# unclearness/vacancy

Hardware: AMD Instinct MI355X
Metric: Mvoxel*views/s (Carve) (higher is better)
Workload: dtype f32

## Files before the change

### include/vacancy_hip.h

```cpp
#ifndef VACANCY_HIP_H_
#define VACANCY_HIP_H_

#include <stdint.h>

#ifdef __cplusplus
extern "C" {
#endif

typedef enum vcy_status {
  VCY_OK = 0,
  VCY_ERR_INVALID_ARG = -1,
  VCY_ERR_NOT_INITIALIZED = -2,
  VCY_ERR_TOO_MANY_VOXELS = -3,
  VCY_ERR_HIP = -4,
  VCY_ERR_NO_DEVICE = -5,
  VCY_ERR_UNSUPPORTED = -6,
  VCY_ERR_INTERNAL = -7
} vcy_status;

enum { VCY_UPDATE_MAX = 0, VCY_UPDATE_WEIGHTED_AVERAGE = 1 };
enum { VCY_INTERP_NN = 0, VCY_INTERP_BILINEAR = 1 };
enum { VCY_OUTSIDE_NONE = 0, VCY_OUTSIDE_MAX = 1 };

typedef struct vcy_update_option {
// ... 127 lines not shown
int vcy_set_param(vcy_ctx* ctx, const char* name, int value);
int vcy_get_param(vcy_ctx* ctx, const char* name, int* value);
int vcy_set_stream(vcy_ctx* ctx, void* hip_stream);
int vcy_get_stream(vcy_ctx* ctx, void** hip_stream_out);
int vcy_sync(vcy_ctx* ctx);
int vcy_timer_begin(vcy_ctx* ctx);
int vcy_timer_end(vcy_ctx* ctx, float* elapsed_ms);

int vcy_last_carve_ms(vcy_ctx* ctx, float* prepass_ms, float* kernel_ms);
int vcy_carve_log(vcy_ctx* ctx, int max_records, float* begin_ms, float* prepass_ms, float* kernel_ms,
                  int32_t* first_chunk, int* n_records, int clear);

int vcy_last_carve_pairs(vcy_ctx* ctx, int64_t* processed, int64_t* total, int64_t* per_layer, int max_layers,
                         int* n_layers);

int vcy_plan_z_slabs(vcy_ctx* ctx, int n_views, const vcy_view* views, const float* const* sdf_device, int n_slabs,
                     int sample_stride, float brick_cost, int32_t* z_bounds, double* layer_cost, int max_layers,
                     int* n_layers);

int vcy_partition_layers(const double* layer_cost, int n_layers, int n_slabs, int nz, int32_t* z_bounds);

int vcy_selftest(vcy_ctx* ctx);

int vcy_measure_bandwidth(int device_id, uint64_t bytes, int reps, double* read_gbs, double* copy_gbs);

typedef struct vcy_clock_probe vcy_clock_probe;
int vcy_clock_probe_start(int device_id, int max_samples, vcy_clock_probe** out);
int vcy_clock_probe_stop(vcy_clock_probe* probe, double* mean_hz, double* settled_hz, double* min_hz, double* max_hz,
                         int* n_samples, double* covered_ms);

// ... 8 lines not shown
```

### vacancy_amd/capi.py

```python
import ctypes as C
import os

_HERE = os.path.dirname(os.path.abspath(__file__))
LIB_PATH = os.environ.get("VCY_HIP_LIB") or os.path.join(_HERE, "csrc", "libvacancy_hip.so")

VCY_OK, VCY_ERR_INVALID_ARG, VCY_ERR_NOT_INITIALIZED, VCY_ERR_TOO_MANY_VOXELS = 0, -1, -2, -3
VCY_ERR_HIP, VCY_ERR_NO_DEVICE, VCY_ERR_UNSUPPORTED, VCY_ERR_INTERNAL = -4, -5, -6, -7
VCY_UPDATE_MAX, VCY_UPDATE_WEIGHTED_AVERAGE = 0, 1
VCY_INTERP_NN, VCY_INTERP_BILINEAR = 0, 1
VCY_OUTSIDE_NONE, VCY_OUTSIDE_MAX = 0, 1


class UpdateOption(C.Structure):
    _fields_ = [
        ("voxel_update", C.c_int32),
        ("sdf_interp", C.c_int32),
        ("update_outside", C.c_int32),
        ("voxel_max_update_num", C.c_int32),
        ("voxel_update_weight", C.c_float),
        ("use_truncation", C.c_int32),
        ("truncation_band", C.c_float),
    ]

    def __init__(self, voxel_update=VCY_UPDATE_MAX, sdf_interp=VCY_INTERP_BILINEAR,
# ... 128 lines not shown
        "vcy_device_free": (C.c_int, [vp, vp]),
        "vcy_device_alloc": (C.c_int, [vp, C.c_int64, P(vp)]),
        "vcy_memcpy_h2d": (C.c_int, [vp, vp, vp, C.c_int64]),
        "vcy_memcpy_d2h": (C.c_int, [vp, vp, vp, C.c_int64]),
        "vcy_reset": (C.c_int, [vp]),
        "vcy_set_param": (C.c_int, [vp, C.c_char_p, C.c_int]),
        "vcy_get_param": (C.c_int, [vp, C.c_char_p, P(C.c_int)]),
        "vcy_set_stream": (C.c_int, [vp, vp]),
        "vcy_get_stream": (C.c_int, [vp, P(vp)]),
        "vcy_sync": (C.c_int, [vp]),
        "vcy_timer_begin": (C.c_int, [vp]),
        "vcy_timer_end": (C.c_int, [vp, P(C.c_float)]),
        "vcy_selftest": (C.c_int, [vp]),
        "vcy_last_carve_ms": (C.c_int, [vp, P(C.c_float), P(C.c_float)]),
        "vcy_last_carve_pairs": (C.c_int, [vp, P(C.c_int64), P(C.c_int64), vp, C.c_int, P(C.c_int)]),
        "vcy_plan_z_slabs": (C.c_int, [vp, C.c_int, P(View), P(vp), C.c_int, C.c_int, C.c_float, vp, vp, C.c_int,
                                       P(C.c_int)]),
        "vcy_last_stream_ms": (C.c_int, [vp, P(C.c_float), P(C.c_float), P(C.c_float)]),
        "vcy_partition_layers": (C.c_int, [vp, C.c_int, C.c_int, C.c_int, vp]),
        "vcy_carve_log": (C.c_int, [vp, C.c_int, vp, vp, vp, vp, P(C.c_int), C.c_int]),
        "vcy_measure_bandwidth": (C.c_int, [C.c_int, C.c_uint64, C.c_int, P(C.c_double), P(C.c_double)]),
        "vcy_clock_probe_start": (C.c_int, [C.c_int, C.c_int, P(vp)]),
        "vcy_clock_probe_stop": (C.c_int, [vp, P(C.c_double), P(C.c_double), P(C.c_double), P(C.c_double), P(C.c_int),
                                           P(C.c_double)]),
        "vcy_last_error": (C.c_char_p, []),
        "vcy_version": (C.c_char_p, []),
    }
    for name, (res, args) in sig.items():
        fn = getattr(lib, name)
        fn.restype = res
# ... 5 lines not shown
```

### vacancy_amd/carver.py

```python
import ctypes as C

import numpy as np

from . import capi
from .capi import CarverOption, Mesh, UpdateOption, View, make_view


def _p(a):
    return a.ctypes.data_as(C.c_void_p)


def _mesh_array(ptr, count, width, dtype):
    if count == 0 or not ptr:
        return np.zeros((0, width), dtype)
    return np.ctypeslib.as_array(ptr, shape=(count * width,)).reshape(count, width).copy()


def last_error():
    return capi.load().vcy_last_error().decode()


class VoxelCarver:
    def __init__(self, option=None, device_id=0, z_range=None):
        self._lib = capi.load()
# ... 277 lines not shown
    def selftest(self):
        return self._lib.vcy_selftest(self._ctx) == 0

    def last_carve_ms(self):
        a, b = C.c_float(), C.c_float()
        assert self._lib.vcy_last_carve_ms(self._ctx, C.byref(a), C.byref(b)) == 0, last_error()
        return a.value, b.value

    def last_carve_pairs(self):
        a, b, n = C.c_int64(), C.c_int64(), C.c_int()
        per = np.zeros(4096, np.int64)
        rc = self._lib.vcy_last_carve_pairs(self._ctx, C.byref(a), C.byref(b), _p(per), len(per), C.byref(n))
        if rc != 0:
            raise RuntimeError(last_error())
        return int(a.value), int(b.value), per[: n.value].copy()

    def plan_z_slabs(self, views, sdf_devs, n_slabs, stride=0, brick_cost=0.0):
        n, arr, ptrs = views if sdf_devs is None else self.prepare_batch(views, sdf_devs)
        bounds = np.zeros(n_slabs + 1, np.int32)
        cost = np.zeros(8192, np.float64)
        nl = C.c_int()
        rc = self._lib.vcy_plan_z_slabs(self._ctx, n, arr, ptrs, int(n_slabs), int(stride), float(brick_cost),
                                        _p(bounds), _p(cost), len(cost), C.byref(nl))
        if rc != 0:
            raise RuntimeError(last_error())
        return [int(z) for z in bounds], cost[: nl.value].copy()

    def carve_log(self, clear=True, max_records=8192):
        b = np.empty(max_records, np.float32)
        p = np.empty(max_records, np.float32)
# ... 168 lines not shown
```

### vacancy_amd/csrc/carve_fused.hip

```cpp
#include <algorithm>
#include <cmath>
#include <cstdlib>
#include <cstring>
#include <map>
#include <mutex>
#include <utility>
#include <type_traits>
#include <vector>

#include "carve_common.h"

namespace vcy {

void launch_fused_counts8(bool big, int update, bool trunc, bool samef, bool checkmax, unsigned grid_x, hipStream_t s,
                          const GridParams& g, const void* views, const float* c2, int nv, const ModeParams& m, int nbx, int nby,
                          int cull, int state_flags, const void* records, int64_t nbricks, float* bmin, const int* wgl,
                          unsigned long long* pcnt, int row_units);
void launch_fused_counts16(bool big, int update, bool trunc, bool samef, bool checkmax, unsigned grid_x, hipStream_t s,
                           const GridParams& g, const void* views, const float* c2, int nv, const ModeParams& m, int nbx, int nby,
                           int cull, int state_flags, const void* records, int64_t nbricks, float* bmin, const int* wgl,
                           unsigned long long* pcnt, int row_units);

namespace {

// ... 374 lines not shown
  const FusedView& fv = views[blockIdx.y];
  const int w = fv.v.width, h = fv.v.height, wq = (fv.wrect[2] - fv.wrect[0]) >> 2;
  const int t = blockIdx.x * 256 + threadIdx.x;
  if (fv.wmax == nullptr || wq <= 0 || t >= wq * (fv.wrect[3] - fv.wrect[1])) return;
  const int yr = t / wq, y = fv.wrect[1] + yr, x0 = fv.wrect[0] + ((t - yr * wq) << 2);
  const float* in = fv.wmax + (NEG ? 2 * (size_t)fv.wmax_plane : (size_t)0);
  const bool vec = (w & 3) == 0 && ((uintptr_t)in & 15) == 0;
  float a[8], b[8], o[4];
  wmax_load8(in + (size_t)y * w, x0, w, vec, a);
  wmax_load8(y + 4 < h ? in + (size_t)(y + 4) * w : nullptr, x0, w, vec, b);
#pragma unroll
  for (int j = 0; j < 4; ++j) o[j] = fmaxf(fmaxf(a[j], a[j + 4]), fmaxf(b[j], b[j + 4]));
  wmax_store4(const_cast<float*>(in) + (size_t)fv.wmax_plane + (size_t)y * w, x0, w, vec, o);
}

template <bool SAMEF, int TQ, bool GEN>
__device__ __forceinline__ TileInfo footprint_of(const FusedView& fv, float xl, float xh, float yl, float yh, float zl_,
                                                 float zh, bool is_ortho, bool outside_max, bool want_bound,
                                                 bool want_lower, float* lower_out = nullptr) {
  const ViewParams& v = fv.v;
  const float xa = fmaxf(fabsf(xl), fabsf(xh)), ya = fmaxf(fabsf(yl), fabsf(yh)), za = fmaxf(fabsf(zl_), fabsf(zh));
  const bool ortho = GEN && is_ortho;
  float p0[3], ax[3], ay[3], az[3], mag[3];
#pragma unroll
  for (int i = 0; i < 3; ++i) {
    p0[i] = v.t[i] + (v.r[i][0] * xl + (v.r[i][1] * yl + v.r[i][2] * zl_));
    ax[i] = v.r[i][0] * (xh - xl);
    ay[i] = v.r[i][1] * (yh - yl);
    az[i] = v.r[i][2] * (zh - zl_);
    mag[i] = fabsf(v.t[i]) + (fabsf(v.r[i][0]) * xa + (fabsf(v.r[i][1]) * ya + fabsf(v.r[i][2]) * za));
  }
  float umin = INFINITY, umax = -INFINITY, wmin = INFINITY, wmax_ = -INFINITY, zmin = INFINITY, zmax = -INFINITY;
  int bad = 0;
  const float fx = v.fx, fy = SAMEF ? v.fx : v.fy;
  float pxy[4][3];
// ... 26 lines not shown
  bad |= !(mag[0] < 0x1p60f) || !(mag[1] < 0x1p60f) || !(mag[2] < 0x1p60f);
  bad |= !(umin > -1.0e6f) || !(umax < 1.0e6f) || !(wmin > -1.0e6f) || !(wmax_ < 1.0e6f);
  const float uabs = fmaxf(fabsf(umin), fabsf(umax)), wabs = fmaxf(fabsf(wmin), fabsf(wmax_));
  float err_u, err_w;
  if (ortho) {
    err_u = 0x1p-21f * mag[0];
    err_w = 0x1p-21f * mag[1];
  } else {
    bad |= !(zmin * 4.0f >= zmax);
    const float iz = 0x1p-21f * __builtin_amdgcn_rcpf(zmin) * 1.0001f;
    err_u = iz * (fx * mag[0] + (uabs + fabsf(v.cx)) * mag[2]) + 0x1p-21f * (uabs + fabsf(v.cx));
    err_w = iz * (fy * mag[1] + (wabs + fabsf(v.cy)) * mag[2]) + 0x1p-21f * (wabs + fabsf(v.cy));
  }
  const float margin = 0.125f;
  bad |= !(err_u <= 0.03125f) || !(err_w <= 0.03125f);
  TileInfo ti;
  ti.lo_x = ti.lo_y = INFINITY;
  ti.hi_x = ti.hi_y = -INFINITY;
  ti.pitchf = 0.0f;
  ti.base = 0;
  ti.tx0 = ti.ty0 = ti.tw = ti.nq = ti.th = 0;
  ti.inv_tw = 1.0f;
  ti.ub = INFINITY;
  ti.sure = 0;
  if (!bad) {
    const int tx0 = max((int)floorf(umin - margin), v.roi_min_xi);
    const int ty0 = max((int)floorf(wmin - margin), v.roi_min_yi);
    const int tx1 = min((int)floorf(umax + margin), v.roi_max_xi);
    const int ty1 = min((int)floorf(wmax_ + margin), v.roi_max_yi);
    const int tw = tx1 - tx0 + 1, th = ty1 - ty0 + 1;
    constexpr bool kRaw = TQ == kTileRaw;
    if (tw > 0 && th > 0 && (kRaw ? (tw <= 15 && th <= 15) : ((tw + 1) * (th + 1) <= kBigPixels))) {
      const bool unclipped = (int)floorf(umin - margin) >= v.roi_min_xi && (int)floorf(wmin - margin) >= v.roi_min_yi &&
                             (int)floorf(umax + margin) < v.roi_max_xi && (int)floorf(wmax_ + margin) < v.roi_max_yi;
      const bool depth_ok = 0x1p-20f * mag[2] <= 0.25f * zmin && zmin >= 0x1p-58f && zmax <= 0x1p58f;
      const int pitch = kRaw ? 16 : tw + 1;
      const bool small_base = ty0 * pitch + tx0 < (1 << 18);
      const bool depth_ok_ortho = zmin > 0x1p-20f * mag[2];
      ti.sure = (unclipped && (ortho ? depth_ok_ortho : depth_ok) && small_base) ? 1 : 0;
      ti.tx0 = tx0;
      ti.ty0 = ty0;
      ti.tw = tw;
      ti.th = th;
      ti.nq = tw * th;
      ti.inv_tw = 1.0f / (float)pitch;
      ti.pitchf = (float)pitch;
      ti.base = -(ty0 * pitch + tx0);
      ti.lo_x = (float)tx0;
      ti.lo_y = (float)ty0;
      ti.hi_x = (tx1 == v.roi_max_xi) ? v.roi_max_x
                                      : __uint_as_float(__float_as_uint((float)(tx1 + 1)) - 1u);
      ti.hi_y = (ty1 == v.roi_max_yi) ? v.roi_max_y
                                      : __uint_as_float(__float_as_uint((float)(ty1 + 1)) - 1u);
      if (want_bound) {
        const int pw = min(tx1 + 1, v.roi_max_xi) - tx0 + 1;
        const int ph = min(ty1 + 1, v.roi_max_yi) - ty0 + 1;
        float m = -INFINITY;
        int has_nan = 0;
        gfloat_ptr wm = (gfloat_ptr)fv.wmax;
        const int L = min(pw, ph) >= 8 ? 3 : 2;
        const int k = 1 << L;
        const int nxw = (pw + k - 1) >> L, nyw = (ph + k - 1) >> L;
        const bool small = nxw <= 3 && nyw <= 3;
        const int ux = __any(small && nxw >= 3) ? 3 : (__any(small && nxw >= 2) ? 2 : 1);
        const int uy = __any(small && nyw >= 3) ? 3 : (__any(small && nyw >= 2) ? 2 : 1);
        if (wm != nullptr) {
          gfloat_ptr lvl = wm + (L == 3 ? (size_t)fv.wmax_plane : (size_t)0);
          const unsigned origin = __umul24((unsigned)v.width, (unsigned)ty0) + (unsigned)tx0 + (L == 3 ? (unsigned)fv.wmax_plane : 0u);
          if (nxw <= 3 && nyw <= 3) {
            float t[9];
#pragma unroll
            for (int bq = 0; bq < 3; ++bq) {
              const unsigned ro = origin + __umul24((unsigned)v.width, (unsigned)min(bq << L, max(ph - k, 0)));
#pragma unroll
              for (int aq = 0; aq < 3; ++aq) {
                t[3 * bq + aq] = -INFINITY;
                if (aq < ux && bq < uy) t[3 * bq + aq] = load_u32_index(wm, ro + (unsigned)min(aq << L, max(pw - k, 0)));
              }
            }
#pragma unroll
            for (int q = 0; q < 9; ++q) m = fmaxf(m, t[q]);
          } else {
            for (int bq = 0; bq < nyw; ++bq) {
              gfloat_ptr row = lvl + (unsigned)v.width * (unsigned)(ty0 + min(bq << L, max(ph - k, 0)));
              for (int aq = 0; aq < nxw; ++aq) m = fmaxf(m, row[tx0 + min(aq << L, max(pw - k, 0))]);
            }
          }
        } else {
          gfloat_ptr img = (gfloat_ptr)v.sdf;
          for (int j = 0; j < ph; ++j) {
            gfloat_ptr row = img + ((unsigned)v.width * (unsigned)(ty0 + j) + (unsigned)tx0);
            for (int i = 0; i < pw; ++i) {
              const float t = row[i];
              has_nan |= !(fabsf(t) <= 3.402823466e+38f);
              m = fmaxf(m, t);
            }
          }
        }
        if (outside_max && !ti.sure) {
          has_nan |= !(fabsf(v.max_sdf) <= 3.402823466e+38f);
          m = fmaxf(m, v.max_sdf);
        }
        ti.ub = has_nan ? INFINITY : (__builtin_fmaf(fabsf(m), 0x1p-20f, m) + 1.0e-30f);
        if (want_lower && ti.sure && !(ti.ub < -1.0f) && wm != nullptr && fv.has_lower && nxw <= 3 && nyw <= 3) {
          const unsigned origin = __umul24((unsigned)v.width, (unsigned)ty0) + (unsigned)tx0 +
                                  (L == 3 ? 3u : 2u) * (unsigned)fv.wmax_plane;
          float t[9], mneg = -INFINITY;
#pragma unroll
          for (int bq = 0; bq < 3; ++bq) {
            const unsigned ro = origin + __umul24((unsigned)v.width, (unsigned)min(bq << L, max(ph - k, 0)));
#pragma unroll
            for (int aq = 0; aq < 3; ++aq) {
              t[3 * bq + aq] = -INFINITY;
              if (aq < ux && bq < uy) t[3 * bq + aq] = load_u32_index(wm, ro + (unsigned)min(aq << L, max(pw - k, 0)));
            }
          }
#pragma unroll
          for (int q = 0; q < 9; ++q) mneg = fmaxf(mneg, t[q]);
          const float neg_lb = __builtin_fmaf(fabsf(mneg), 0x1p-20f, mneg);
          if (neg_lb <= 1.0f) ti.sure |= 2;
          if (lower_out) *lower_out = -neg_lb;
        }
      }
    }
  }
  return ti;
}

__device__ __forceinline__ FusedView load_fused_view(const FusedView* __restrict__ views, int vi) {
  static_assert(sizeof(FusedView) % 4 == 0, "FusedView is fetched dword by dword");
  constexpr int kViewDwords = (int)(sizeof(FusedView) / 4);
  typedef const uint32_t __attribute__((address_space(1))) * gu32_ptr;
  gu32_ptr src = (gu32_ptr)views + (size_t)vi * kViewDwords;
  uint32_t raw[kViewDwords];
#pragma unroll
  for (int q = 0; q < kViewDwords; ++q) raw[q] = src[q];
#pragma unroll
  for (int q = 0; q < kViewDwords; ++q) asm volatile("" : "+v"(raw[q]));
// ... 92 lines not shown
};
BlockDecode make_block_decode(unsigned grid_x, int nbx, int nby) {
  BlockDecode d;
  d.total = (int)grid_x;
  d.layer = nbx * nby;
  d.q = d.layer >> 3;
  d.rem = d.layer & 7;
  d.dealt = 8 * d.q * (int)(grid_x / (unsigned)std::max(d.layer, 1));
  d.dq = make_fast_div_u32((uint32_t)std::max(d.q, 1));
  d.drem = make_fast_div_u32((uint32_t)std::max(d.rem, 1));
  d.dnbx = make_fast_div_u32((uint32_t)std::max(nbx, 1));
  d.dnby = make_fast_div_u32((uint32_t)std::max(nby, 1));
  return d;
}

template <bool SAMEF, bool GEN>
__global__ __launch_bounds__(256) void footprint_records_kernel(GridParams g, const FusedView* __restrict__ views,
                                                                int nbw, int nby, int64_t nbricks, ModeParams mode,
                                                                int want_bound, int want_lower,
                                                                FootprintRecord* __restrict__ records,
                                                                FastDivU32 div_nbw, FastDivU32 div_nby, int small32) {
  const int64_t brick = (int64_t)blockIdx.x * 256 + threadIdx.x;
  if (brick >= nbricks) return;
  const int vi = blockIdx.y;
  int bxw, by, bz;
  if (small32) {
    const uint32_t b32 = (uint32_t)brick;
    const uint32_t rowb = fast_div_u32(b32, div_nbw);
    bxw = (int)(b32 - rowb * (uint32_t)nbw);
    const uint32_t zz = fast_div_u32(rowb, div_nby);
    by = (int)(rowb - zz * (uint32_t)nby);
    bz = (int)zz;
  } else {
    bxw = (int)(brick % nbw);
    const int64_t rowb = brick / nbw;
    by = (int)(rowb % nby);
    bz = (int)(rowb / nby);
  }
  const int x_lo = min(bxw * WX, g.nx - 1), x_hi = min(bxw * WX + WX - 1, g.nx - 1);
  const int y_hi = min(by * BY + BY - 1, g.ny - 1), z_hi = min(bz * BZ + BZ - 1, g.nz_local - 1);
  const FusedView& fv = views[vi];
  gfloat_ptr ax = (gfloat_ptr)g.px, ay = (gfloat_ptr)g.py, az = (gfloat_ptr)g.pz;
  const TileInfo ti = footprint_of<SAMEF, kTileRaw, GEN>(
      fv, load_u32_index(ax, (unsigned)x_lo), load_u32_index(ax, (unsigned)x_hi), load_u32_index(ay, (unsigned)(by * BY)),
      load_u32_index(ay, (unsigned)y_hi), load_u32_index(az, (unsigned)(g.z0 + bz * BZ)),
      load_u32_index(az, (unsigned)(g.z0 + z_hi)), mode.ortho != 0, mode.outside == VCY_OUTSIDE_MAX, want_bound != 0,
      want_lower != 0);
  records[(int64_t)vi * nbricks + brick] = pack_footprint(ti, fv.v);
}

constexpr int kLiveThreads = 1024;
constexpr int kLiveEntryWords = 2 + 2 * kWgWaves;
__global__ __launch_bounds__(kLiveThreads) void live_workgroups_kernel(const FootprintRecord* __restrict__ recs, int64_t nbricks,
                                                                       int nviews, const float* __restrict__ bmin, int trunc,
                                                                       int nbx, int nby, int nbw, int nwg, int* __restrict__ list,
                                                                       int unit_bricks, int entry_words) {
  __shared__ int wave_count[kLiveThreads / 64];
  __shared__ int block_base;
  const int wg = blockIdx.x * kLiveThreads + threadIdx.x;
  bool live = false;
  unsigned live_bricks = 0u;
  FootprintRecord rec0[kWgWaves];
  for (int j = 0; j < kWgWaves; ++j) rec0[j].w0 = 0u, rec0[j].w1 = 0u;
// ... 1368 lines not shown
  }
  const int row_views = c->row_kernel < 0 ? kRowMaxViews : std::min(c->row_kernel, kRowMaxViews);
  const bool rows = !big && !checkmax && (c->nx & (WX - 1)) == 0 && n_views <= row_views && c->prologue_mode != 1;
  const int nseg = (nbw + kRowBricks - 1) / kRowBricks;
  const bool one_view = c->one_view && n_views == 1 && !rows && !big && !checkmax && c->prologue_mode != 1;
  const bool coop_ok = (kWgWaves == 4 || kWgWaves == 8) && (c->nx & (WX - 1)) == 0 && !big && !rows;
  const int coop_views = c->fresh ? 1 : (u.voxel_update == VCY_UPDATE_MAX ? 1 : kLiveListMaxViews);
  const bool coop = coop_ok && (c->coop_store > 0 || (c->coop_store < 0 && n_views <= coop_views));
  const bool nt = coop && c->nt_store != 0;
  const int state_flags_base = (c->fresh ? 1 : 0) | (c->cnt_implied ? 2 : 0) | (c->brick_min_valid && !c->fresh ? 4 : 0) |
                               (coop ? 8 : 0) | (nt ? 16 : 0);
  const int64_t layer_bricks = (int64_t)nbw * nby;
  int chunk_layers = nbz;
  const int64_t rec_cap = c->record_bytes_max > 0 ? c->record_bytes_max : kRecordBytesMax;
  const bool in_kernel_prologue = !big && c->prologue_mode == 1;
  if (!big && !in_kernel_prologue) {
    const int64_t per_layer = layer_bricks * n_views * (int64_t)sizeof(FootprintRecord);
    const int64_t cap = rec_cap;
    chunk_layers = (int)std::max<int64_t>(1, std::min<int64_t>(nbz, cap / std::max<int64_t>(per_layer, 1)));
    const size_t need = (size_t)(per_layer * chunk_layers);
    if (c->records_bytes < need) {
      VCY_HIP_CHECK(hipStreamSynchronize(c->stream));
      if (c->d_records) (void)hipFree(c->d_records);
      c->d_records = nullptr;
      c->records_bytes = 0;
      VCY_HIP_CHECK(hipMalloc(&c->d_records, need));
      c->records_bytes = need;
    }
  }
  if (c->count_pairs) {
// ... 16 lines not shown
    gc.sdf = g.sdf + (int64_t)l0 * BZ * c->slice;
    gc.cnt = (char*)g.cnt + (int64_t)l0 * BZ * c->slice * c->cnt_bytes;
    gc.z0 = g.z0 + l0 * BZ;
    gc.nz_local = std::min(layers * BZ, nzl - l0 * BZ);
    const int64_t nbricks = layer_bricks * layers;
    FootprintRecord* recs = in_kernel_prologue ? nullptr : (FootprintRecord*)c->d_records;
    float* bmin = c->d_brick_min ? c->d_brick_min + (int64_t)l0 * layer_bricks : nullptr;
    unsigned long long* pcnt = c->count_pairs && c->d_pair_count ? c->d_pair_count + l0 : nullptr;
    if (timed && l0 > 0) {
      stamp = carve_log_open(c, false);
      if (stamp >= 0) VCY_HIP_CHECK(hipEventRecord(c->carve_log[stamp].ev[0], c->stream));
    }
    if (!big && !in_kernel_prologue) {
      const dim3 pgrid((unsigned)((nbricks + 255) / 256), (unsigned)n_views);
      const FastDivU32 div_nbw = make_fast_div_u32((uint32_t)nbw), div_nby = make_fast_div_u32((uint32_t)nby);
#define VCY_PREPASS(SF, GN)                                                                                       \
  hipLaunchKernelGGL((footprint_records_kernel<SF, GN>), pgrid, dim3(256), 0, c->stream, gc, d_views, nbw, nby,   \
                     nbricks, m, need_bound ? 1 : 0, want_lower ? 1 : 0, recs, div_nbw, div_nby,                  \
                     nbricks < 0xffffffffLL ? 1 : 0)
      if (samef) { if (gen) VCY_PREPASS(true, true); else VCY_PREPASS(true, false); }
      else { if (gen) VCY_PREPASS(false, true); else VCY_PREPASS(false, false); }
#undef VCY_PREPASS
      VCY_HIP_CHECK(hipGetLastError());
    }
    const int unit_bricks = rows ? kRowBricks : kWgWaves;
    const int units_x = rows ? nseg : nbx;
    const dim3 grid((unsigned)((int64_t)units_x * nby * layers));
    auto groups_of = [&](unsigned units) {
      return rows ? dim3((units + kRowWaves - 1) / kRowWaves) : dim3(units);
    };
    dim3 launch_grid = rows ? dim3(8u * ((grid.x + 8u * kRowWaves - 1) / (8u * kRowWaves))) : grid;
    const int* wgl = nullptr;
    int list_entry_words = 0;
    const bool have_min = u.voxel_update == VCY_UPDATE_MAX && (state_flags_base & 4) != 0 && bmin != nullptr;
    const bool list_pays = c->h_live_hint == nullptr || c->h_live_hint[1] <= 0 ||
                           (double)c->h_live_hint[0] < 0.6 * (double)c->h_live_hint[1];
    ++c->live_list_age;
    if (!big && recs != nullptr && c->use_live_list && need_bound && !c->fresh && n_views <= kLiveListMaxViews && (m.trunc != 0 || have_min) &&
// ... 186 lines not shown
```

### vacancy_amd/csrc/vcy_api.hip

```cpp
#include <algorithm>
#include <cstdarg>
#include <cstring>
#include <chrono>
#include <limits>
#include <mutex>
#include <thread>
#include <vector>

#include "vcy_internal.h"
#include "build_id.h"

namespace vcy {

static thread_local std::string g_last_error;

void set_error(const char* fmt, ...) {
  char buf[1024];
  va_list ap;
  va_start(ap, fmt);
  vsnprintf(buf, sizeof(buf), fmt, ap);
  va_end(ap);
  g_last_error = buf;
}

// ... 543 lines not shown
    return VCY_OK;
  }
  if (std::strcmp(name, "recordbytes") == 0) {
    c->record_bytes_max = value > 0 ? value : 0;
    return VCY_OK;
  }
  if (std::strcmp(name, "livelist") == 0) {
    c->use_live_list = value != 0;
    return VCY_OK;
  }
  if (std::strcmp(name, "prologue") == 0) {
    if (value < 0 || value > 2) return VCY_ERR_INVALID_ARG;
    c->prologue_mode = value;
    return VCY_OK;
  }
  if (std::strcmp(name, "livesync") == 0) {
    c->live_sync = value != 0;
    return VCY_OK;
  }
  if (std::strcmp(name, "coopstore") == 0) {
    c->coop_store = value < 0 ? -1 : (value != 0 ? 1 : 0);
    return VCY_OK;
  }
  if (std::strcmp(name, "listrecords") == 0) {
    c->list_records = value != 0;
    return VCY_OK;
  }
  if (std::strcmp(name, "eagerstate") == 0) {
    c->eager_state = value < 0 ? -1 : (value != 0 ? 1 : 0);
    return VCY_OK;
// ... 42 lines not shown
  else if (std::strcmp(name, "cull") == 0) *value = c->use_cull ? 1 : 0;
  else if (std::strcmp(name, "tile") == 0) *value = c->tile_mode;
  else if (std::strcmp(name, "defer") == 0) *value = c->defer ? 1 : 0;
  else if (std::strcmp(name, "shortdiv") == 0) *value = c->use_short_div ? 1 : 0;
  else if (std::strcmp(name, "div_level") == 0) *value = c->last_div_level;
  else if (std::strcmp(name, "mcsweep") == 0) *value = c->mc_sweep ? 1 : 0;
  else if (std::strcmp(name, "mcskip") == 0) *value = c->mc_skip;
  else if (std::strcmp(name, "rowkernel") == 0) *value = c->row_kernel;
  else if (std::strcmp(name, "ntstore") == 0) *value = c->nt_store;
  else if (std::strcmp(name, "oneview") == 0) *value = c->one_view;
  else if (std::strcmp(name, "eagerstate") == 0) *value = c->eager_state;
  else if (std::strcmp(name, "listrecords") == 0) *value = c->list_records;
  else if (std::strcmp(name, "mcdirect") == 0) *value = (int)std::min<int64_t>(c->mc_direct_bytes, 0x7fffffff);
  else if (std::strcmp(name, "livelist") == 0) *value = c->use_live_list ? 1 : 0;
  else if (std::strcmp(name, "prologue") == 0) *value = c->prologue_mode;
  else if (std::strcmp(name, "coopstore") == 0) *value = c->coop_store;
  else if (std::strcmp(name, "livesync") == 0) *value = c->live_sync ? 1 : 0;
  else if (std::strcmp(name, "brick_min_valid") == 0) *value = c->brick_min_valid && !c->fresh ? 1 : 0;
  else if (std::strcmp(name, "meshkeys") == 0) *value = c->mesh_keys ? 1 : 0;
  else if (std::strcmp(name, "lazycount") == 0) *value = c->lazy_count ? 1 : 0;
  else if (std::strcmp(name, "carvetimer") == 0) *value = c->time_carve ? 1 : 0;
  else if (std::strcmp(name, "carvelog_dropped") == 0) *value = c->carve_log_dropped;
  else if (std::strcmp(name, "count_bytes") == 0) *value = c->cnt_bytes;
  else if (std::strcmp(name, "count_bytes_final") == 0) *value = c->cnt_bytes_wire;
  else {
    set_error("unknown parameter %s", name);
    return VCY_ERR_INVALID_ARG;
  }
  return VCY_OK;
}
// ... 79 lines not shown
    return VCY_ERR_INVALID_ARG;
  }
  VCY_HIP_CHECK(hipSetDevice(c->device));
  const int nbz = (c->nz_local() + 7) / 8;
  std::vector<unsigned long long> h((size_t)nbz, 0ull);
  VCY_HIP_CHECK(hipMemcpyAsync(h.data(), c->d_pair_count, sizeof(unsigned long long) * (size_t)nbz, hipMemcpyDeviceToHost, c->stream));
  VCY_HIP_CHECK(hipStreamSynchronize(c->stream));
  int64_t sum = 0;
  for (int l = 0; l < nbz; ++l) {
    sum += (int64_t)h[(size_t)l];
    if (per_layer && l < max_layers) per_layer[l] = (int64_t)h[(size_t)l];
  }
  if (processed) *processed = sum;
  if (total) *total = (int64_t)((c->nx + 7) / 8) * ((c->ny + 7) / 8) * nbz * c->pair_count_views;
  if (n_layers) *n_layers = nbz;
  return VCY_OK;
}

int vcy_partition_layers(const double* layer_cost, int n_layers, int n_slabs, int nz, int32_t* z_bounds) {
  if (!layer_cost || !z_bounds || n_layers < 1 || n_slabs < 1 || n_slabs > n_layers || nz <= (n_layers - 1) * 8 ||
      nz > n_layers * 8) {
    set_error("vcy_partition_layers: invalid argument");
    return VCY_ERR_INVALID_ARG;
  }
  if (n_slabs > 1 && n_layers > 1 && nz - (n_layers - 1) * 8 == 1 && n_slabs > n_layers - 1) {
    set_error("vcy_partition_layers: the last layer is a single slice and cannot be a slab of its own");
    return VCY_ERR_INVALID_ARG;
  }
  for (int l = 0; l < n_layers; ++l)
    if (!(layer_cost[l] >= 0.0) || !(layer_cost[l] < 1e280)) {
// ... 888 lines not shown
```

### vacancy_amd/csrc/vcy_internal.h

```cpp
#pragma once

#include <hip/hip_runtime.h>

#include <cstdint>
#include <cstdio>
#include <string>
#include <utility>
#include <vector>

#include "vacancy_hip.h"

namespace vcy {

void set_error(const char* fmt, ...);

#define VCY_HIP_CHECK(expr)                                                        \
  do {                                                                             \
    hipError_t _e = (expr);                                                        \
    if (_e != hipSuccess) {                                                        \
      ::vcy::set_error("%s failed: %s (%s:%d)", #expr, hipGetErrorString(_e),      \
                       __FILE__, __LINE__);                                        \
      return VCY_ERR_HIP;                                                          \
    }                                                                              \
  } while (0)
// ... 79 lines not shown
  std::vector<CarveStamp> carve_log;
  int carve_log_n = 0;
  int carve_log_last = 0;
  int carve_log_dropped = 0;
  bool carve_log_last_dropped = false;
  int* h_live_hint = nullptr;
  int64_t live_list_age = 0;
  bool use_live_list = true;
  bool live_sync = true;
  int coop_store = -1;
  bool count_pairs = false;
  unsigned long long* d_pair_count = nullptr;
  int pair_count_layers = 0, pair_count_views = 0;
  int64_t record_bytes_max = 0;
  int prologue_mode = 0;
  void* d_records = nullptr;
  size_t records_bytes = 0;
  float* d_wmax = nullptr;
  size_t wmax_bytes = 0;
  bool fused_ortho = false;
  void* h_fused_stage[2] = {nullptr, nullptr};
  hipEvent_t ev_fused_stage[2] = {nullptr, nullptr};
  size_t fused_stage_bytes = 0;
  int fused_stage_idx = 0;
  bool fused_cache_valid = false;
  std::vector<char> fused_cache_vp;
  const float* fused_cache_wmax = nullptr;
  void* fused_cache_at = nullptr;
  bool fused_cache_bound = false, fused_cache_lower = false, fused_cache_ortho = false, fused_cache_samef = true;
  int fused_cache_max_quads = 0;
  int fused_cache_z[2] = {0, 0};
  void* d_stream_pool = nullptr;
// ... 73 lines not shown
```

Baseline: 4.286 million.

## Process two views per thread in footprint prepass to batch window loads

Adds a prepass kernel variant where each thread handles a brick for two views at once. It decodes the brick and loads its extent once, then issues both views' max-window loads before reducing them, so more independent memory loads are in flight per thread. The footprint code is split into helpers to support this, and the new variant is the default, selectable through a 'prepass' parameter. It also adds a debug API for copying records back to the host. In exchange the kernel uses more registers per thread and the grid has half as many view blocks.

New measurement: 4.339 million, median of 6. 1.01x the previous value.

```diff
diff --git a/include/vacancy_hip.h b/include/vacancy_hip.h
--- a/include/vacancy_hip.h
+++ b/include/vacancy_hip.h
@@ -165,6 +165,8 @@
 int vcy_last_carve_pairs(vcy_ctx* ctx, int64_t* processed, int64_t* total, int64_t* per_layer, int max_layers,
                          int* n_layers);
 
+int vcy_debug_copy_records(vcy_ctx* ctx, void* dst, int64_t max_bytes, int64_t* bytes);
+
 int vcy_plan_z_slabs(vcy_ctx* ctx, int n_views, const vcy_view* views, const float* const* sdf_device, int n_slabs,
                      int sample_stride, float brick_cost, int32_t* z_bounds, double* layer_cost, int max_layers,
                      int* n_layers);
diff --git a/vacancy_amd/capi.py b/vacancy_amd/capi.py
--- a/vacancy_amd/capi.py
+++ b/vacancy_amd/capi.py
@@ -166,6 +166,7 @@
         "vcy_selftest": (C.c_int, [vp]),
         "vcy_last_carve_ms": (C.c_int, [vp, P(C.c_float), P(C.c_float)]),
         "vcy_last_carve_pairs": (C.c_int, [vp, P(C.c_int64), P(C.c_int64), vp, C.c_int, P(C.c_int)]),
+        "vcy_debug_copy_records": (C.c_int, [vp, vp, C.c_int64, P(C.c_int64)]),
         "vcy_plan_z_slabs": (C.c_int, [vp, C.c_int, P(View), P(vp), C.c_int, C.c_int, C.c_float, vp, vp, C.c_int,
                                        P(C.c_int)]),
         "vcy_last_stream_ms": (C.c_int, [vp, P(C.c_float), P(C.c_float), P(C.c_float)]),
diff --git a/vacancy_amd/carver.py b/vacancy_amd/carver.py
--- a/vacancy_amd/carver.py
+++ b/vacancy_amd/carver.py
@@ -315,6 +315,18 @@
         if rc != 0:
             raise RuntimeError(last_error())
         return int(a.value), int(b.value), per[: n.value].copy()
+
+    def debug_records(self):
+        n = C.c_int64()
+        rc = self._lib.vcy_debug_copy_records(self._ctx, None, 0, C.byref(n))
+        if rc != 0:
+            raise RuntimeError(last_error())
+        out = np.zeros((n.value // 8, 2), np.uint32)
+        got = C.c_int64()
+        rc = self._lib.vcy_debug_copy_records(self._ctx, _p(out), out.nbytes, C.byref(got))
+        if rc != 0 or got.value != n.value:
+            raise RuntimeError(last_error())
+        return out
 
     def plan_z_slabs(self, views, sdf_devs, n_slabs, stride=0, brick_cost=0.0):
         n, arr, ptrs = views if sdf_devs is None else self.prepare_batch(views, sdf_devs)
diff --git a/vacancy_amd/csrc/carve_fused.hip b/vacancy_amd/csrc/carve_fused.hip
--- a/vacancy_amd/csrc/carve_fused.hip
+++ b/vacancy_amd/csrc/carve_fused.hip
@@ -412,11 +412,10 @@
   wmax_store4(const_cast<float*>(in) + (size_t)fv.wmax_plane + (size_t)y * w, x0, w, vec, o);
 }
 
+
 template <bool SAMEF, int TQ, bool GEN>
-__device__ __forceinline__ TileInfo footprint_of(const FusedView& fv, float xl, float xh, float yl, float yh, float zl_,
-                                                 float zh, bool is_ortho, bool outside_max, bool want_bound,
-                                                 bool want_lower, float* lower_out = nullptr) {
-  const ViewParams& v = fv.v;
+__device__ __forceinline__ bool footprint_rect(const ViewParams& v, float xl, float xh, float yl, float yh, float zl_,
+                                               float zh, bool is_ortho, TileInfo& ti, int& tx1_out, int& ty1_out) {
   const float xa = fmaxf(fabsf(xl), fabsf(xh)), ya = fmaxf(fabsf(yl), fabsf(yh)), za = fmaxf(fabsf(zl_), fabsf(zh));
   const bool ortho = GEN && is_ortho;
   float p0[3], ax[3], ay[3], az[3], mag[3];
@@ -473,7 +472,6 @@
   }
   const float margin = 0.125f;
   bad |= !(err_u <= 0.03125f) || !(err_w <= 0.03125f);
-  TileInfo ti;
   ti.lo_x = ti.lo_y = INFINITY;
   ti.hi_x = ti.hi_y = -INFINITY;
   ti.pitchf = 0.0f;
@@ -482,6 +480,7 @@
   ti.inv_tw = 1.0f;
   ti.ub = INFINITY;
   ti.sure = 0;
+  tx1_out = ty1_out = 0;
   if (!bad) {
     const int tx0 = max((int)floorf(umin - margin), v.roi_min_xi);
     const int ty0 = max((int)floorf(wmin - margin), v.roi_min_yi);
@@ -511,76 +510,125 @@
                                       : __uint_as_float(__float_as_uint((float)(tx1 + 1)) - 1u);
       ti.hi_y = (ty1 == v.roi_max_yi) ? v.roi_max_y
                                       : __uint_as_float(__float_as_uint((float)(ty1 + 1)) - 1u);
-      if (want_bound) {
-        const int pw = min(tx1 + 1, v.roi_max_xi) - tx0 + 1;
-        const int ph = min(ty1 + 1, v.roi_max_yi) - ty0 + 1;
-        float m = -INFINITY;
-        int has_nan = 0;
-        gfloat_ptr wm = (gfloat_ptr)fv.wmax;
-        const int L = min(pw, ph) >= 8 ? 3 : 2;
-        const int k = 1 << L;
-        const int nxw = (pw + k - 1) >> L, nyw = (ph + k - 1) >> L;
-        const bool small = nxw <= 3 && nyw <= 3;
-        const int ux = __any(small && nxw >= 3) ? 3 : (__any(small && nxw >= 2) ? 2 : 1);
-        const int uy = __any(small && nyw >= 3) ? 3 : (__any(small && nyw >= 2) ? 2 : 1);
-        if (wm != nullptr) {
-          gfloat_ptr lvl = wm + (L == 3 ? (size_t)fv.wmax_plane : (size_t)0);
-          const unsigned origin = __umul24((unsigned)v.width, (unsigned)ty0) + (unsigned)tx0 + (L == 3 ? (unsigned)fv.wmax_plane : 0u);
-          if (nxw <= 3 && nyw <= 3) {
-            float t[9];
-#pragma unroll
-            for (int bq = 0; bq < 3; ++bq) {
-              const unsigned ro = origin + __umul24((unsigned)v.width, (unsigned)min(bq << L, max(ph - k, 0)));
-#pragma unroll
-              for (int aq = 0; aq < 3; ++aq) {
-                t[3 * bq + aq] = -INFINITY;
-                if (aq < ux && bq < uy) t[3 * bq + aq] = load_u32_index(wm, ro + (unsigned)min(aq << L, max(pw - k, 0)));
-              }
-            }
-#pragma unroll
-            for (int q = 0; q < 9; ++q) m = fmaxf(m, t[q]);
-          } else {
-            for (int bq = 0; bq < nyw; ++bq) {
-              gfloat_ptr row = lvl + (unsigned)v.width * (unsigned)(ty0 + min(bq << L, max(ph - k, 0)));
-              for (int aq = 0; aq < nxw; ++aq) m = fmaxf(m, row[tx0 + min(aq << L, max(pw - k, 0))]);
-            }
-          }
-        } else {
-          gfloat_ptr img = (gfloat_ptr)v.sdf;
-          for (int j = 0; j < ph; ++j) {
-            gfloat_ptr row = img + ((unsigned)v.width * (unsigned)(ty0 + j) + (unsigned)tx0);
-            for (int i = 0; i < pw; ++i) {
-              const float t = row[i];
-              has_nan |= !(fabsf(t) <= 3.402823466e+38f);
-              m = fmaxf(m, t);
-            }
-          }
-        }
-        if (outside_max && !ti.sure) {
-          has_nan |= !(fabsf(v.max_sdf) <= 3.402823466e+38f);
-          m = fmaxf(m, v.max_sdf);
-        }
-        ti.ub = has_nan ? INFINITY : (__builtin_fmaf(fabsf(m), 0x1p-20f, m) + 1.0e-30f);
-        if (want_lower && ti.sure && !(ti.ub < -1.0f) && wm != nullptr && fv.has_lower && nxw <= 3 && nyw <= 3) {
-          const unsigned origin = __umul24((unsigned)v.width, (unsigned)ty0) + (unsigned)tx0 +
-                                  (L == 3 ? 3u : 2u) * (unsigned)fv.wmax_plane;
-          float t[9], mneg = -INFINITY;
-#pragma unroll
-          for (int bq = 0; bq < 3; ++bq) {
-            const unsigned ro = origin + __umul24((unsigned)v.width, (unsigned)min(bq << L, max(ph - k, 0)));
-#pragma unroll
-            for (int aq = 0; aq < 3; ++aq) {
-              t[3 * bq + aq] = -INFINITY;
-              if (aq < ux && bq < uy) t[3 * bq + aq] = load_u32_index(wm, ro + (unsigned)min(aq << L, max(pw - k, 0)));
-            }
-          }
-#pragma unroll
-          for (int q = 0; q < 9; ++q) mneg = fmaxf(mneg, t[q]);
-          const float neg_lb = __builtin_fmaf(fabsf(mneg), 0x1p-20f, mneg);
-          if (neg_lb <= 1.0f) ti.sure |= 2;
-          if (lower_out) *lower_out = -neg_lb;
-        }
-      }
+      tx1_out = tx1;
+      ty1_out = ty1;
+      return true;
+    }
+  }
+  return false;
+}
+
+struct WindowPlan {
+  int L, pw, ph, nxw, nyw;
+};
+__device__ __forceinline__ WindowPlan window_plan(const ViewParams& v, int tx0, int ty0, int tx1, int ty1) {
+  WindowPlan p;
+  p.pw = min(tx1 + 1, v.roi_max_xi) - tx0 + 1;
+  p.ph = min(ty1 + 1, v.roi_max_yi) - ty0 + 1;
+  p.L = min(p.pw, p.ph) >= 8 ? 3 : 2;
+  const int k = 1 << p.L;
+  p.nxw = (p.pw + k - 1) >> p.L;
+  p.nyw = (p.ph + k - 1) >> p.L;
+  return p;
+}
+
+__device__ __forceinline__ void window_loads(gfloat_ptr wm, unsigned origin, unsigned width, const WindowPlan& p,
+                                             int ux, int uy, bool on, float t[9]) {
+  const int k = 1 << p.L;
+#pragma unroll
+  for (int bq = 0; bq < 3; ++bq) {
+    const unsigned ro = origin + __umul24(width, (unsigned)min(bq << p.L, max(p.ph - k, 0)));
+#pragma unroll
+    for (int aq = 0; aq < 3; ++aq) {
+      t[3 * bq + aq] = -INFINITY;
+      if (aq < ux && bq < uy) t[3 * bq + aq] = load_u32_index(wm, on ? ro + (unsigned)min(aq << p.L, max(p.pw - k, 0)) : 0u);
+    }
+  }
+}
+
+__device__ __forceinline__ void window_counts(const WindowPlan& p, bool small, int& ux, int& uy) {
+  ux = __any(small && p.nxw >= 3) ? 3 : (__any(small && p.nxw >= 2) ? 2 : 1);
+  uy = __any(small && p.nyw >= 3) ? 3 : (__any(small && p.nyw >= 2) ? 2 : 1);
+}
+
+__device__ __forceinline__ float window_max_slow(const FusedView& fv, int tx0, int ty0, const WindowPlan& p, int* has_nan) {
+  const ViewParams& v = fv.v;
+  gfloat_ptr wm = (gfloat_ptr)fv.wmax;
+  float m = -INFINITY;
+  if (wm != nullptr) {
+    const int k = 1 << p.L;
+    gfloat_ptr lvl = wm + (p.L == 3 ? (size_t)fv.wmax_plane : (size_t)0);
+    for (int bq = 0; bq < p.nyw; ++bq) {
+      gfloat_ptr row = lvl + (unsigned)v.width * (unsigned)(ty0 + min(bq << p.L, max(p.ph - k, 0)));
+      for (int aq = 0; aq < p.nxw; ++aq) m = fmaxf(m, row[tx0 + min(aq << p.L, max(p.pw - k, 0))]);
+    }
+  } else {
+    gfloat_ptr img = (gfloat_ptr)v.sdf;
+    for (int j = 0; j < p.ph; ++j) {
+      gfloat_ptr row = img + ((unsigned)v.width * (unsigned)(ty0 + j) + (unsigned)tx0);
+      for (int i = 0; i < p.pw; ++i) {
+        const float t = row[i];
+        *has_nan |= !(fabsf(t) <= 3.402823466e+38f);
+        m = fmaxf(m, t);
+      }
+    }
+  }
+  return m;
+}
+
+__device__ __forceinline__ float footprint_ub(const ViewParams& v, float m, int has_nan, bool outside_max, int sure) {
+  if (outside_max && !sure) {
+    has_nan |= !(fabsf(v.max_sdf) <= 3.402823466e+38f);
+    m = fmaxf(m, v.max_sdf);
+  }
+  return has_nan ? INFINITY : (__builtin_fmaf(fabsf(m), 0x1p-20f, m) + 1.0e-30f);
+}
+
+__device__ __forceinline__ bool wants_lower(const FusedView& fv, const TileInfo& ti, const WindowPlan& p) {
+  return ti.sure && !(ti.ub < -1.0f) && fv.wmax != nullptr && fv.has_lower && p.nxw <= 3 && p.nyw <= 3;
+}
+__device__ __forceinline__ unsigned lower_origin(const FusedView& fv, int tx0, int ty0, const WindowPlan& p) {
+  return __umul24((unsigned)fv.v.width, (unsigned)ty0) + (unsigned)tx0 + (p.L == 3 ? 3u : 2u) * (unsigned)fv.wmax_plane;
+}
+__device__ __forceinline__ float neg_lower_bound(const float t[9]) {
+  float mneg = -INFINITY;
+#pragma unroll
+  for (int q = 0; q < 9; ++q) mneg = fmaxf(mneg, t[q]);
+  return __builtin_fmaf(fabsf(mneg), 0x1p-20f, mneg);
+}
+
+template <bool SAMEF, int TQ, bool GEN>
+__device__ __forceinline__ TileInfo footprint_of(const FusedView& fv, float xl, float xh, float yl, float yh, float zl_,
+                                                 float zh, bool is_ortho, bool outside_max, bool want_bound,
+                                                 bool want_lower, float* lower_out = nullptr) {
+  const ViewParams& v = fv.v;
+  TileInfo ti;
+  int tx1, ty1;
+  if (footprint_rect<SAMEF, TQ, GEN>(v, xl, xh, yl, yh, zl_, zh, is_ortho, ti, tx1, ty1) && want_bound) {
+    const int tx0 = ti.tx0, ty0 = ti.ty0;
+    const WindowPlan p = window_plan(v, tx0, ty0, tx1, ty1);
+    float m = -INFINITY;
+    int has_nan = 0;
+    gfloat_ptr wm = (gfloat_ptr)fv.wmax;
+    const bool small = p.nxw <= 3 && p.nyw <= 3;
+    int ux, uy;
+    window_counts(p, small, ux, uy);
+    if (wm != nullptr && small) {
+      float t[9];
+      window_loads(wm, __umul24((unsigned)v.width, (unsigned)ty0) + (unsigned)tx0 + (p.L == 3 ? (unsigned)fv.wmax_plane : 0u),
+                   (unsigned)v.width, p, ux, uy, true, t);
+#pragma unroll
+      for (int q = 0; q < 9; ++q) m = fmaxf(m, t[q]);
+    } else {
+      m = window_max_slow(fv, tx0, ty0, p, &has_nan);
+    }
+    ti.ub = footprint_ub(v, m, has_nan, outside_max, ti.sure);
+    if (want_lower && wants_lower(fv, ti, p)) {
+      float t[9];
+      window_loads(wm, lower_origin(fv, tx0, ty0, p), (unsigned)v.width, p, ux, uy, true, t);
+      const float neg_lb = neg_lower_bound(t);
+      if (neg_lb <= 1.0f) ti.sure |= 2;
+      if (lower_out) *lower_out = -neg_lb;
     }
   }
   return ti;
@@ -703,16 +751,8 @@
   return d;
 }
 
-template <bool SAMEF, bool GEN>
-__global__ __launch_bounds__(256) void footprint_records_kernel(GridParams g, const FusedView* __restrict__ views,
-                                                                int nbw, int nby, int64_t nbricks, ModeParams mode,
-                                                                int want_bound, int want_lower,
-                                                                FootprintRecord* __restrict__ records,
-                                                                FastDivU32 div_nbw, FastDivU32 div_nby, int small32) {
-  const int64_t brick = (int64_t)blockIdx.x * 256 + threadIdx.x;
-  if (brick >= nbricks) return;
-  const int vi = blockIdx.y;
-  int bxw, by, bz;
+__device__ __forceinline__ void decode_brick(int64_t brick, int nbw, int nby, FastDivU32 div_nbw, FastDivU32 div_nby,
+                                             int small32, int& bxw, int& by, int& bz) {
   if (small32) {
     const uint32_t b32 = (uint32_t)brick;
     const uint32_t rowb = fast_div_u32(b32, div_nbw);
@@ -726,16 +766,118 @@
     by = (int)(rowb % nby);
     bz = (int)(rowb / nby);
   }
+}
+
+__device__ __forceinline__ void brick_extent(const GridParams& g, int bxw, int by, int bz, float ext[6]) {
   const int x_lo = min(bxw * WX, g.nx - 1), x_hi = min(bxw * WX + WX - 1, g.nx - 1);
   const int y_hi = min(by * BY + BY - 1, g.ny - 1), z_hi = min(bz * BZ + BZ - 1, g.nz_local - 1);
+  gfloat_ptr ax = (gfloat_ptr)g.px, ay = (gfloat_ptr)g.py, az = (gfloat_ptr)g.pz;
+  ext[0] = load_u32_index(ax, (unsigned)x_lo);
+  ext[1] = load_u32_index(ax, (unsigned)x_hi);
+  ext[2] = load_u32_index(ay, (unsigned)(by * BY));
+  ext[3] = load_u32_index(ay, (unsigned)y_hi);
+  ext[4] = load_u32_index(az, (unsigned)(g.z0 + bz * BZ));
+  ext[5] = load_u32_index(az, (unsigned)(g.z0 + z_hi));
+}
+
+template <bool SAMEF, bool GEN>
+__global__ __launch_bounds__(256) void footprint_records_kernel(GridParams g, const FusedView* __restrict__ views,
+                                                                int nbw, int nby, int64_t nbricks, ModeParams mode,
+                                                                int want_bound, int want_lower,
+                                                                FootprintRecord* __restrict__ records,
+                                                                FastDivU32 div_nbw, FastDivU32 div_nby, int small32) {
+  const int64_t brick = (int64_t)blockIdx.x * 256 + threadIdx.x;
+  if (brick >= nbricks) return;
+  const int vi = blockIdx.y;
+  int bxw, by, bz;
+  decode_brick(brick, nbw, nby, div_nbw, div_nby, small32, bxw, by, bz);
   const FusedView& fv = views[vi];
-  gfloat_ptr ax = (gfloat_ptr)g.px, ay = (gfloat_ptr)g.py, az = (gfloat_ptr)g.pz;
-  const TileInfo ti = footprint_of<SAMEF, kTileRaw, GEN>(
-      fv, load_u32_index(ax, (unsigned)x_lo), load_u32_index(ax, (unsigned)x_hi), load_u32_index(ay, (unsigned)(by * BY)),
-      load_u32_index(ay, (unsigned)y_hi), load_u32_index(az, (unsigned)(g.z0 + bz * BZ)),
-      load_u32_index(az, (unsigned)(g.z0 + z_hi)), mode.ortho != 0, mode.outside == VCY_OUTSIDE_MAX, want_bound != 0,
-      want_lower != 0);
+  float e[6];
+  brick_extent(g, bxw, by, bz, e);
+  const TileInfo ti = footprint_of<SAMEF, kTileRaw, GEN>(fv, e[0], e[1], e[2], e[3], e[4], e[5], mode.ortho != 0,
+                                                         mode.outside == VCY_OUTSIDE_MAX, want_bound != 0, want_lower != 0);
   records[(int64_t)vi * nbricks + brick] = pack_footprint(ti, fv.v);
+}
+
+constexpr int kPrepassViews = 2;
+
+template <bool SAMEF, bool GEN, int VT>
+__global__ __launch_bounds__(256) void footprint_records_vt_kernel(GridParams g, const FusedView* __restrict__ views,
+                                                                   int nviews, int nbw, int nby, int64_t nbricks,
+                                                                   ModeParams mode, int want_bound, int want_lower,
+                                                                   FootprintRecord* __restrict__ records,
+                                                                   FastDivU32 div_nbw, FastDivU32 div_nby, int small32) {
+  const int64_t brick = (int64_t)blockIdx.x * 256 + threadIdx.x;
+  if (brick >= nbricks) return;
+  const int v0 = blockIdx.y * VT;
+  const int nv = min(VT, nviews - v0);
+  int bxw, by, bz;
+  decode_brick(brick, nbw, nby, div_nbw, div_nby, small32, bxw, by, bz);
+  float e[6];
+  brick_extent(g, bxw, by, bz, e);
+  TileInfo ti[VT];
+  WindowPlan p[VT];
+  bool has[VT];
+#pragma unroll
+  for (int k = 0; k < VT; ++k) {
+    if (k < nv) {
+      const ViewParams& v = views[v0 + k].v;
+      int tx1, ty1;
+      has[k] = footprint_rect<SAMEF, kTileRaw, GEN>(v, e[0], e[1], e[2], e[3], e[4], e[5], mode.ortho != 0, ti[k], tx1, ty1);
+      p[k] = window_plan(v, ti[k].tx0, ti[k].ty0, tx1, ty1);
+    }
+  }
+  if (want_bound) {
+    float t[VT][9];
+    int ux[VT], uy[VT];
+#pragma unroll
+    for (int k = 0; k < VT; ++k) {
+      if (k < nv) {
+        const FusedView& fv = views[v0 + k];
+        const bool small = has[k] && p[k].nxw <= 3 && p[k].nyw <= 3;
+        window_counts(p[k], small, ux[k], uy[k]);
+        if (fv.wmax != nullptr)
+          window_loads((gfloat_ptr)fv.wmax,
+                       __umul24((unsigned)fv.v.width, (unsigned)ti[k].ty0) + (unsigned)ti[k].tx0 +
+                           (p[k].L == 3 ? (unsigned)fv.wmax_plane : 0u),
+                       (unsigned)fv.v.width, p[k], ux[k], uy[k], small, t[k]);
+      }
+    }
+#pragma unroll
+    for (int k = 0; k < VT; ++k) {
+      if (k < nv && has[k]) {
+        const FusedView& fv = views[v0 + k];
+        float m = -INFINITY;
+        int has_nan = 0;
+        if (fv.wmax != nullptr && p[k].nxw <= 3 && p[k].nyw <= 3) {
+#pragma unroll
+          for (int q = 0; q < 9; ++q) m = fmaxf(m, t[k][q]);
+        } else {
+          m = window_max_slow(fv, ti[k].tx0, ti[k].ty0, p[k], &has_nan);
+        }
+        ti[k].ub = footprint_ub(fv.v, m, has_nan, mode.outside == VCY_OUTSIDE_MAX, ti[k].sure);
+      }
+    }
+    if (want_lower) {
+      bool lo[VT];
+#pragma unroll
+      for (int k = 0; k < VT; ++k) {
+        if (k < nv) {
+          const FusedView& fv = views[v0 + k];
+          lo[k] = has[k] && wants_lower(fv, ti[k], p[k]);
+          if (fv.wmax != nullptr && fv.has_lower)
+            window_loads((gfloat_ptr)fv.wmax, lower_origin(fv, ti[k].tx0, ti[k].ty0, p[k]), (unsigned)fv.v.width, p[k],
+                         ux[k], uy[k], lo[k], t[k]);
+        }
+      }
+#pragma unroll
+      for (int k = 0; k < VT; ++k)
+        if (k < nv && lo[k] && neg_lower_bound(t[k]) <= 1.0f) ti[k].sure |= 2;
+    }
+  }
+#pragma unroll
+  for (int k = 0; k < VT; ++k)
+    if (k < nv) records[(int64_t)(v0 + k) * nbricks + brick] = pack_footprint(ti[k], views[v0 + k].v);
 }
 
 constexpr int kLiveThreads = 1024;
@@ -2134,6 +2276,7 @@
   int chunk_layers = nbz;
   const int64_t rec_cap = c->record_bytes_max > 0 ? c->record_bytes_max : kRecordBytesMax;
   const bool in_kernel_prologue = !big && c->prologue_mode == 1;
+  c->records_last_bytes = 0;
   if (!big && !in_kernel_prologue) {
     const int64_t per_layer = layer_bricks * n_views * (int64_t)sizeof(FootprintRecord);
     const int64_t cap = rec_cap;
@@ -2180,14 +2323,23 @@
     if (!big && !in_kernel_prologue) {
       const dim3 pgrid((unsigned)((nbricks + 255) / 256), (unsigned)n_views);
       const FastDivU32 div_nbw = make_fast_div_u32((uint32_t)nbw), div_nby = make_fast_div_u32((uint32_t)nby);
-#define VCY_PREPASS(SF, GN)                                                                                       \
-  hipLaunchKernelGGL((footprint_records_kernel<SF, GN>), pgrid, dim3(256), 0, c->stream, gc, d_views, nbw, nby,   \
-                     nbricks, m, need_bound ? 1 : 0, want_lower ? 1 : 0, recs, div_nbw, div_nby,                  \
-                     nbricks < 0xffffffffLL ? 1 : 0)
+      const dim3 vgrid(pgrid.x, (unsigned)((n_views + kPrepassViews - 1) / kPrepassViews));
+#define VCY_PREPASS(SF, GN)                                                                                        \
+  do {                                                                                                             \
+    if (c->prepass_mode == 0)                                                                                      \
+      hipLaunchKernelGGL((footprint_records_kernel<SF, GN>), pgrid, dim3(256), 0, c->stream, gc, d_views, nbw,     \
+                         nby, nbricks, m, need_bound ? 1 : 0, want_lower ? 1 : 0, recs, div_nbw, div_nby,          \
+                         nbricks < 0xffffffffLL ? 1 : 0);                                                           \
+    else                                                                                                           \
+      hipLaunchKernelGGL((footprint_records_vt_kernel<SF, GN, kPrepassViews>), vgrid, dim3(256), 0, c->stream, gc, \
+                         d_views, n_views, nbw, nby, nbricks, m, need_bound ? 1 : 0, want_lower ? 1 : 0, recs,     \
+                         div_nbw, div_nby, nbricks < 0xffffffffLL ? 1 : 0);                                         \
+  } while (0)
       if (samef) { if (gen) VCY_PREPASS(true, true); else VCY_PREPASS(true, false); }
       else { if (gen) VCY_PREPASS(false, true); else VCY_PREPASS(false, false); }
 #undef VCY_PREPASS
       VCY_HIP_CHECK(hipGetLastError());
+      c->records_last_bytes = nbricks * n_views * (int64_t)sizeof(FootprintRecord);
     }
     const int unit_bricks = rows ? kRowBricks : kWgWaves;
     const int units_x = rows ? nseg : nbx;
diff --git a/vacancy_amd/csrc/vcy_api.hip b/vacancy_amd/csrc/vcy_api.hip
--- a/vacancy_amd/csrc/vcy_api.hip
+++ b/vacancy_amd/csrc/vcy_api.hip
@@ -581,6 +581,11 @@
     c->prologue_mode = value;
     return VCY_OK;
   }
+  if (std::strcmp(name, "prepass") == 0) {
+    if (value < 0 || value > 1) return VCY_ERR_INVALID_ARG;
+    c->prepass_mode = value;
+    return VCY_OK;
+  }
   if (std::strcmp(name, "livesync") == 0) {
     c->live_sync = value != 0;
     return VCY_OK;
@@ -653,6 +658,7 @@
   else if (std::strcmp(name, "mcdirect") == 0) *value = (int)std::min<int64_t>(c->mc_direct_bytes, 0x7fffffff);
   else if (std::strcmp(name, "livelist") == 0) *value = c->use_live_list ? 1 : 0;
   else if (std::strcmp(name, "prologue") == 0) *value = c->prologue_mode;
+  else if (std::strcmp(name, "prepass") == 0) *value = c->prepass_mode;
   else if (std::strcmp(name, "coopstore") == 0) *value = c->coop_store;
   else if (std::strcmp(name, "livesync") == 0) *value = c->live_sync ? 1 : 0;
   else if (std::strcmp(name, "brick_min_valid") == 0) *value = c->brick_min_valid && !c->fresh ? 1 : 0;
@@ -762,6 +768,20 @@
   if (processed) *processed = sum;
   if (total) *total = (int64_t)((c->nx + 7) / 8) * ((c->ny + 7) / 8) * nbz * c->pair_count_views;
   if (n_layers) *n_layers = nbz;
+  return VCY_OK;
+}
+
+int vcy_debug_copy_records(vcy_ctx* c, void* dst, int64_t max_bytes, int64_t* bytes) {
+  if (!c) return VCY_ERR_NOT_INITIALIZED;
+  if (!bytes || (max_bytes > 0 && !dst)) return VCY_ERR_INVALID_ARG;
+  VCY_HIP_CHECK(hipSetDevice(c->device));
+  { const int rcf = flush_pending(c); if (rcf != VCY_OK) return rcf; }
+  *bytes = c->d_records ? c->records_last_bytes : 0;
+  const int64_t n = std::min<int64_t>(*bytes, std::max<int64_t>(max_bytes, 0));
+  if (n > 0) {
+    VCY_HIP_CHECK(hipMemcpyAsync(dst, c->d_records, (size_t)n, hipMemcpyDeviceToHost, c->stream));
+    VCY_HIP_CHECK(hipStreamSynchronize(c->stream));
+  }
   return VCY_OK;
 }
 
diff --git a/vacancy_amd/csrc/vcy_internal.h b/vacancy_amd/csrc/vcy_internal.h
--- a/vacancy_amd/csrc/vcy_internal.h
+++ b/vacancy_amd/csrc/vcy_internal.h
@@ -117,8 +117,10 @@
   int pair_count_layers = 0, pair_count_views = 0;
   int64_t record_bytes_max = 0;
   int prologue_mode = 0;
+  int prepass_mode = 1;
   void* d_records = nullptr;
   size_t records_bytes = 0;
+  int64_t records_last_bytes = 0;
   float* d_wmax = nullptr;
   size_t wmax_bytes = 0;
   bool fused_ortho = false;
```
